# 54rt1n/shardmerge

Hardware: AMD Instinct MI355X
Metric: merged-weight GB/s per GPU + % HBM roofline, Llama-3-70B 3-way FFT merge (higher is better)
Workload: dtype f32; 1 GPU; Llama-3-70B block tensors, this rank's 1/8 slice (9 per block x 10 blocks), K=3 finetunes, bf16 in/out, resident in HBM; workload_id=llama3-70b-slice, k=3, parallelism=tensor-partition x1 (no data-path collective), streams_per_gpu=8

## Files before the change

### shardmerge_amd/csrc/sm_capi.inc

```

struct smhip_ctx {
    smhip::Pipeline<SM_BACKEND> pipe;
    explicit smhip_ctx(int device) : pipe(device) {}
};

#define SM_GUARD(ctx)                      \
    if (!(ctx)) return SMHIP_ERR_ARG;      \
    (ctx)->pipe.err.clear();
#define SM_FINISH(ctx, rc)                                                        \
    do {                                                                          \
        int rc__ = (rc);                                                          \
        if (rc__ == SMHIP_OK && !(ctx)->pipe.be.ok()) {                           \
            (ctx)->pipe.err = (ctx)->pipe.be.error();                             \
            rc__ = SMHIP_ERR_HIP;                                                 \
        }                                                                         \
        return rc__;                                                              \
    } while (0)

template <class Desc, class Scalars>
static int delta_tensor_check(smhip_ctx* ctx, const char* op, const Desc* d, const void* out, const float* delta_out,
                              bool need_base, Scalars scalars) {
    auto bad = [&](const char* what) { return ctx->pipe.fail(SMHIP_ERR_ARG, std::string(op) + ": " + what); };
    if (!d) return bad("null descriptor");
    if (d->k < 1 || d->k > SMHIP_MAX_MODELS) return bad("k out of range (1..16)");
// ... 336 lines not shown
    SM_GUARD(ctx);
    if (!x || !norm_out) return ctx->pipe.fail(SMHIP_ERR_ARG, "bad argument");
    if (dtype < SMHIP_BF16 || dtype > SMHIP_F32) return ctx->pipe.fail(SMHIP_ERR_ARG, "bad dtype");
    ctx->pipe.stream = stream;
    const int rc0 = ctx->pipe.reserve(1, 1);
    if (rc0) SM_FINISH(ctx, rc0);
    smhip::SigDesc sg{x, base, dtype, 1.f};
    double out = 0;
    if (!ctx->pipe.run_serial_norms(&sg, 1, n, &out))
        return ctx->pipe.fail(SMHIP_ERR_ARG, "reference_cpu norm: inputs must be 16-byte aligned");
    *norm_out = (float)out;
    SM_FINISH(ctx, SMHIP_OK);
}

int smhip_debug_option(smhip_ctx* ctx, const char* key, long value) {
    SM_GUARD(ctx);
    if (key && std::string(key) == "aten_overlap") { ctx->pipe.aten_overlap = value != 0; return SMHIP_OK; }
    if (key && std::string(key) == "emf_max_sample") { ctx->pipe.emf_max_sample = value >= 1 && value <= 4096 ? (int)value : smhip::EMF_MAX_SAMPLE; return SMHIP_OK; }
    if (key && std::string(key) == "aten_serial") { ctx->pipe.aten_serial = value != 0; return SMHIP_OK; }
    if (key && std::string(key) == "class_norms") { ctx->pipe.class_norms_mode = value >= 0 && value <= 2 ? (int)value : 1; return SMHIP_OK; }
    if (key && std::string(key) == "cand_cap") { ctx->pipe.debug_cand_cap = value > 0 ? (uint32_t)value : 0u; return SMHIP_OK; }
    if (key && std::string(key) == "sel_chunks") { ctx->pipe.debug_sel_chunks = value > 0 ? (uint32_t)value : 0u; return SMHIP_OK; }
    if (key && std::string(key) == "sel_flush_always") { ctx->pipe.debug_flush_always = value != 0; return SMHIP_OK; }
    if (key && std::string(key) == "fuse_norms") { ctx->pipe.fuse_norms = value != 0; return SMHIP_OK; }
    if (key && std::string(key) == "noise_seed") { ctx->pipe.noise_seed_base = (uint32_t)value; return SMHIP_OK; }
    if (key && std::string(key) == "spectral_intermediates") { ctx->pipe.spectral_inter = value != 0; return SMHIP_OK; }
    if (key && std::string(key) == "fuse_spec_norm") { ctx->pipe.fuse_spec_norm = value != 0; return SMHIP_OK; }
    if (key && std::string(key) == "sel_wgs_per_cu") { ctx->pipe.sel_wgs_per_cu = value > 0 ? (int)value : 5; return SMHIP_OK; }
    if (key && std::string(key) == "pair1d") { ctx->pipe.pair1d_enabled = value != 0; return SMHIP_OK; }
    if (key && std::string(key) == "spec_cull") { ctx->pipe.spec_cull = value != 0; return SMHIP_OK; }
    if (key && std::string(key) == "spec_min_bins") { ctx->pipe.spec_min_bins = value >= 0 ? (size_t)value : (size_t)1 << 20; return SMHIP_OK; }
    if (key && std::string(key) == "dftp_pairs") { ctx->pipe.dftp_pairs_enabled = value != 0; return SMHIP_OK; }
    if (key && std::string(key) == "f2s_pair") { ctx->pipe.f2s_pair = value != 0; return SMHIP_OK; }
    if (key && std::string(key) == "f1_multi") { ctx->pipe.f1_multi = value != 0; return SMHIP_OK; }
    if (key && std::string(key) == "force_bluestein") { ctx->pipe.debug_force_bluestein = value != 0; return SMHIP_OK; }
    if (key && std::string(key) == "force_split") { ctx->pipe.debug_force_split = value > 1 && value <= smhip::DFTP_MAX_P ? (int)value : 0; return SMHIP_OK; }
    if (key && std::string(key) == "fold_columns") { ctx->pipe.fold_enabled = value != 0; return SMHIP_OK; }
    if (key && std::string(key) == "della_slab_rows") { ctx->pipe.della_slab_rows = value > 0 ? (size_t)value : 0; return SMHIP_OK; }
    if (key && std::string(key) == "fold_min_rows") { ctx->pipe.fold_min_rows = value > 0 ? (int)value : SM_FOLD_MIN_ROWS; return SMHIP_OK; }
    return ctx->pipe.fail(SMHIP_ERR_ARG, "unknown debug option");
}

int smhip_debug_query(smhip_ctx* ctx, const char* key, long* value) {
    SM_GUARD(ctx);
    if (!key || !value) return SMHIP_ERR_ARG;
    if (std::string(key) == "spec_hit") { *value = ctx->pipe.last_spec_verdict(); SM_FINISH(ctx, SMHIP_OK); }
    if (std::string(key) == "spec_checked" || std::string(key) == "spec_hits") {
        unsigned long long c = 0, h = 0;
        ctx->pipe.spec_totals(&c, &h);
        *value = (long)(std::string(key) == "spec_hits" ? h : c);
        SM_FINISH(ctx, SMHIP_OK);
    }
    if (std::string(key) == "aten_fast" || std::string(key) == "aten_group" || std::string(key) == "aten_slow") {
        unsigned long long v3[3];
        ctx->pipe.aten_stats(1, v3);
        *value = (long)v3[std::string(key) == "aten_fast" ? 0 : std::string(key) == "aten_group" ? 1 : 2];
        SM_FINISH(ctx, SMHIP_OK);
    }
    return ctx->pipe.fail(SMHIP_ERR_ARG, "unknown debug query");
}

int smhip_profile_enable(smhip_ctx* ctx, int on) { SM_GUARD(ctx); ctx->pipe.be.profile_enable(on != 0); return SMHIP_OK; }
int smhip_profile_reset(smhip_ctx* ctx) { SM_GUARD(ctx); ctx->pipe.be.profile_reset(); return SMHIP_OK; }
int smhip_profile_count(smhip_ctx* ctx) { return ctx ? ctx->pipe.be.profile_count() : 0; }
int smhip_profile_get(smhip_ctx* ctx, int i, const char** name, uint64_t* launches, double* total_ms) {
    SM_GUARD(ctx);
    return ctx->pipe.be.profile_get(i, name, launches, total_ms) ? SMHIP_OK : SMHIP_ERR_ARG;
}

}
```

### shardmerge_amd/csrc/sm_kernels.hpp

```cpp
#pragma once
#include <cmath>
#include <cstring>

#include "fft_engine.hpp"
#include "sm_aten_core.hpp"

namespace smhip {

struct cf4 { float x, y, z, w; };
struct u32x4 { uint32_t x, y, z, w; };

enum { DT_BF16 = 0, DT_F16 = 1, DT_F32 = 2 };

struct SigDesc {
    const void* x;
    const void* base;
    int dtype;
    float prescale;
};

SM_HD uint32_t umax(uint32_t a, uint32_t b) { return a > b ? a : b; }
SM_HD float u2f(uint32_t u) { float f; memcpy(&f, &u, 4); return f; }
SM_HD uint32_t f2u(float f) { uint32_t u; memcpy(&u, &f, 4); return u; }
SM_HD float bf16_to_f(uint32_t h) { return u2f(h << 16); }
// ... 882 lines not shown
    }
}

#ifndef SM_COL_THREADS
#define SM_COL_THREADS 512
#endif
constexpr int f2_bins_for(int T, int N = 1 << 30) {
    if (T == 64 && N <= 256) return 8;
    return (SM_COL_THREADS / (2 * T)) > 1 ? (SM_COL_THREADS / (2 * T) > 8 ? 8 : SM_COL_THREADS / (2 * T)) : 1;
}
#ifndef SM_I1_THREADS
constexpr int i1_bins_for(int T) { return 2; }
#else
constexpr int i1_bins_for(int T) { return (SM_I1_THREADS / T) > 2 ? ((SM_I1_THREADS / T) > 16 ? 16 : (SM_I1_THREADS / T)) : 2; }
#endif
template <class P> constexpr int f2_bins() { if constexpr (P::is_static) return f2_bins_for(P::T, P::N); else return 1; }
template <class P> constexpr int i1_bins() { if constexpr (P::is_static) return i1_bins_for(P::T); else return 2; }

struct F2SParams {
    FftPlanDev plan;
    const cf4* t1;
    int pitch4;
    int R, C, Cb;
    int role_a;
    float scale;
    float* re; float* im;
    unsigned long long* hist;
    int slab, Cb_real, Rfull;
    size_t slab_elems;
    double* im_partials;
    SliceGrid sl;
    int two;
    const cf4* t1_2; int role_a_2; float scale_2; float* re_2;
};
template <class P> constexpr int f2s_groups() {
    if constexpr (P::is_static) return f2_nsig_for(P::T) == 2 ? 2 * f2_bins_for(P::T, P::N) : 1; else return 1;
}

#ifndef SM_F2S_ILV
#define SM_F2S_ILV 1
#endif
constexpr int F2S_ILV = SM_F2S_ILV;
#ifndef SM_F2S_DIRECT
#define SM_F2S_DIRECT 0
#endif
template <class P, int G> constexpr int f2s_direct() {
    if constexpr (!P::is_static) return 0;
    else {
        constexpr int R0 = P::radix(0);
        constexpr bool ok = F2S_ILV == 1 && (G == 1 || G == 2) && P::npass >= 2 && P::T % 2 == 0 && R0 % 2 == 0 &&
                            (P::N / R0) % 2 == 0 && (EMAX / R0) * R0 * P::T >= P::N;
        return ok ? (SM_F2S_DIRECT & 3) : 0;
    }
}
template <class P, int G, bool FOLD = false, class Ex>
SM_HD void k_f2s(Ex& ex, const F2SParams& p) {
    if constexpr (FOLD && !fold_col_plan<P>()) { return; } else {
    typename Ex::template State<FftState> st;
    ex.init(st);
    float* lds = ex.lds() + LDS_SCRATCH_FLOATS;
    const FftPlanDev& pl = p.plan;
    const int T = plan_T<P>(pl), R = plan_N<P>(pl);
    const int LF = plan_lds<P>(pl);
    constexpr int XG = G >= 8 ? 1 : 8 / G;
    int bid_in_slice;
    const int slice = slice_of(ex, p.sl, bid_in_slice);
    int sig2 = 0;
    const int lbid = p.two ? pick_signal(2, bid_in_slice, XG, sig2) : xcd_remap(bid_in_slice, XG);
    const cf4* const t1 = (sig2 ? p.t1_2 : p.t1) + slice * p.sl.t1_stride;
    const size_t pl_off = slice * p.sl.plane_stride;
    const int role_a_ = sig2 ? p.role_a_2 : p.role_a;
    const float scale_ = sig2 ? p.scale_2 : p.scale;
    float* const re_ = sig2 ? p.re_2 : p.re;
    const int kbase = lbid * G;
    if (kbase >= p.Cb) {
        if (p.im_partials) ex.each(st, [&](int tid, FftState&) { if (tid == 0) p.im_partials[ex.bid()] = 0.0; });
        return;
    }
    const int nthreads = G * T;
    const int half = R / 2;
    uint32_t* lhist = (uint32_t*)(lds + G * LF);

    constexpr int DIRECT = f2s_direct<P, G>();
    if constexpr ((DIRECT & 1) != 0) {
        constexpr int R0 = P::radix(0), MB0 = EMAX / R0, nb0 = P::N / R0;
        ex.each(st, [&](int tid, FftState& s) {
            const int g = tid / T, t = tid % T;
            const int k2 = kbase + g;
            const int kc = k2 < p.Cb ? k2 : p.Cb - 1;
            const int par = t & 1;
            static_for<0, MB0>([&](auto m_c) {
                constexpr int m = decltype(m_c)::value;
                const bool live = (t + m * T) < nb0 && k2 < p.Cb;
                static_for<0, R0 / 2>([&](auto q_c) {
                    constexpr int q = decltype(q_c)::value;
                    const int pm = live ? (t >> 1) + m * (T / 2) + q * nb0 + par * (nb0 / 2) : 0;
                    cf4 v;
#if defined(SM_DIAG_NOMEM)
                    v = cf4{(float)q, (float)t, 1.f, (float)kc};
#else
                    if constexpr (FOLD) v = t1[(size_t)(kc / p.slab) * p.slab_elems + (size_t)pm * p.slab + (kc % p.slab)];
                    else v = t1[(size_t)pm * p.pitch4 + kc];
#endif
                    s.xr[m * R0 + 2 * q] = live ? v.x : 0.f; s.xi[m * R0 + 2 * q] = live ? v.y : 0.f;
                    s.xr[m * R0 + 2 * q + 1] = live ? v.z : 0.f; s.xi[m * R0 + 2 * q + 1] = live ? v.w : 0.f;
                });
// ... 55 lines not shown
#pragma unroll
                for (int c = 0; c < 4; ++c) {
                    const int k1 = 4 * (t + u * T) + c;
                    if (k1 < R) o[4 * u + c] = l[lpad(k1)];
                }
            }
        });

    ex.each(st, [&](int tid, FftState& s) {
        const int g = tid / T, t = tid % T;
        const int k2 = kbase + g;
        s.red[0] = 0.0;
        if (k2 >= p.Cb) return;
        const float sc = scale_;
        size_t poff = (size_t)k2 * R;
        int kreal = k2;
        if constexpr (FOLD) { kreal = fold_bin(k2, p.slab, p.Cb_real, R, p.Rfull, poff); if (kreal < 0) return; }
        const uint32_t w = (uint32_t)bin_weight(kreal, p.C);
        float* dre = re_ + pl_off + poff;
        float* dim = p.im + pl_off + poff;
        float imsq = 0.f;
        if constexpr ((DIRECT & 2) != 0) {
            constexpr int RL = P::radix(P::npass - 1), MBL = EMAX / RL, NsL = P::N / RL;
            static_for<0, MBL>([&](auto m_c) {
                constexpr int m = decltype(m_c)::value;
                const int j = t + m * T;
                if (j < NsL) {
                    static_for<0, RL>([&](auto i_c) {
                        constexpr int i = decltype(i_c)::value, e = m * RL + i;
                        const float vr = s.xr[e] * sc;
#if defined(SM_DIAG_NOMEM)
                        if (vr == 12345.678f)
#endif
                        dre[j + i * NsL] = vr;
                        if (role_a_) {
                            const float vi = s.xi[e] * sc;
#if defined(SM_DIAG_NOMEM)
                            if (vi == 12345.678f)
#endif
                            dim[j + i * NsL] = vi;
                            imsq += vi * vi;
                        }
                        if (p.hist) ex.lds_atomic_add(&lhist[(f2u(vr) & 0x7fffffffu) >> 20], w);
                    });
                }
            });
        } else
#pragma unroll
        for (int u = 0; u < EMAX / 4; ++u) {
            const int k0 = 4 * (t + u * T);
            if (k0 + 3 < R && (R & 3) == 0) {
                cf4 vr = {s.xr[4 * u] * sc, s.xr[4 * u + 1] * sc, s.xr[4 * u + 2] * sc, s.xr[4 * u + 3] * sc};
#if defined(SM_DIAG_NOMEM)
                if (vr.x == 12345.678f)
#endif
                *(cf4*)(dre + k0) = vr;
                if (role_a_) {
                    cf4 vi = {s.xi[4 * u] * sc, s.xi[4 * u + 1] * sc, s.xi[4 * u + 2] * sc, s.xi[4 * u + 3] * sc};
#if defined(SM_DIAG_NOMEM)
                    if (vi.x == 12345.678f)
#endif
                    *(cf4*)(dim + k0) = vi;
                    imsq += vi.x * vi.x + vi.y * vi.y + vi.z * vi.z + vi.w * vi.w;
                }
            } else {
#pragma unroll
                for (int c = 0; c < 4; ++c) {
                    if (k0 + c < R) {
                        dre[k0 + c] = s.xr[4 * u + c] * sc;
                        if (role_a_) { const float vi = s.xi[4 * u + c] * sc; dim[k0 + c] = vi; imsq += vi * vi; }
                    }
                }
            }
            if (p.hist) {
#pragma unroll
                for (int c = 0; c < 4; ++c) {
                    if (k0 + c < R) {
                        const uint32_t key = f2u(s.xr[4 * u + c] * sc) & 0x7fffffffu;
                        ex.lds_atomic_add(&lhist[key >> 20], w);
                    }
                }
            }
        }
        s.red[0] = (double)imsq * (double)w;
    });
    if (p.hist) {
        ex.sync();
        ex.each(st, [&](int tid, FftState&) {
            for (int h = tid; h < HIST1_BINS; h += nthreads) {
                const uint32_t v = lhist[h];
                if (v) ex.global_atomic_add(&p.hist[h], (unsigned long long)v);
            }
        });
    }
    if (p.im_partials) {
        ex.sync();
        ex.template block_sum<1>(st, [&](const double* tot) { p.im_partials[ex.bid()] = tot[0]; });
    }
    }
}

template <class Ex>
SM_HD void k_f2_r1(Ex& ex, const F2Params& p) {
// ... 2747 lines not shown
```

### shardmerge_amd/csrc/sm_pipeline.hpp

```cpp
#pragma once
#include <algorithm>
#include <cmath>
#include <cstdio>
#include <map>
#include <string>
#include <vector>

#include "../../include/shardmerge_hip.h"
#include "sm_kernels.hpp"
#include "sm_aten_norm.hpp"
#include "sm_bluestein.hpp"
#include "sm_lora.hpp"
#include "sm_ties.hpp"
#include "sm_dare.hpp"
#include "sm_breadcrumbs.hpp"
#include "sm_geo.hpp"
#include "sm_sce.hpp"
#include "sm_della.hpp"

namespace smhip {

#define SM_KERNEL_TAG(Tag, ParamsT, NAME, CALL)                                      \
    struct Tag {                                                                     \
        using Params = ParamsT;                                                      \
// ... 289 lines not shown
};

struct ProfEntry { std::string name; uint64_t launches = 0; double ms = 0; };

inline size_t round_up(size_t v, size_t m) { return (v + m - 1) / m * m; }

struct PairOut {
    void* out = nullptr; int out_mode = OUT_F32;
    const void* base = nullptr; int base_dtype = DT_BF16;
    float post = 1.f;
    int ifft_policy = 1;
};

template <class B>
class Pipeline {
  public:
    B be;
    std::string err;
    void* stream = nullptr;
    uint32_t debug_cand_cap = 0;
    uint32_t debug_sel_chunks = 0;
    bool debug_flush_always = false;
    bool spec_cull = true;
    size_t spec_min_bins = 1 << 20;
    bool dftp_pairs_enabled = true;
    int debug_force_split = 0;
    int sel_wgs_per_cu = 5;
    bool safe_select = false;
    uint32_t noise_seed_base = 0;
    bool spectral_inter = true;
    bool f2s_pair = true;
    size_t f2s_pair_max_bins = (size_t)64 << 20;
    bool f1_multi = true;
    bool fuse_spec_norm = true;
    float noise_sigma = 1.2e-7f;

    explicit Pipeline(int device) : be(device) {}
    ~Pipeline() {
        for (auto& kv : plans_) if (kv.second.dev.tw) be.free((void*)kv.second.dev.tw);
        for (Buffer* b : {&cand_, &t1_, &small_, &tmpA_, &tmpB_, &tmpC_, &fullS_, &saveR_, &saveI_, &aten_, &emf_, &lora_, &dora_, &ties_}) if (b->p) be.free(b->p);
        for (Buffer& b : pool_) if (b.p) be.free(b.p);
        if (mail_) be.free_host(mail_);
        for (Buffer& b : inter_) if (b.p) be.free(b.p);
        for (Buffer& b : rowspec_) if (b.p) be.free(b.p);
        for (Buffer& b : tr_) if (b.p) be.free(b.p);
        for (auto& kv : rough_tw_) if (kv.second) be.free(kv.second);
        for (auto& kv : blue_) { if (kv.second.chirp) be.free(kv.second.chirp); if (kv.second.filt) be.free(kv.second.filt); }
    }

    int fail(int code, const std::string& msg) { err = msg; return code; }

    int get_plan(int N, FftPlanDev& out) {
        auto it = plans_.find(N);
        if (it == plans_.end()) {
            HostPlan hp;
            int T;
            std::vector<int> rad;
            if (plan_shape(N, T, rad)) {
                hp.ok = true;
                hp.dev.N = N; hp.dev.T = T; hp.dev.npass = (int)rad.size();
                for (int i = 0; i < MAX_PASSES; ++i) hp.dev.radix[i] = i < (int)rad.size() ? rad[i] : 1;
                hp.dev.cx = plan_uses_cx(N) ? 1 : 0;
                hp.dev.lds_floats = hp.dev.cx ? (int)round_up((size_t)2 * (N + (N >> 4) + 1), 32)
                                              : (int)round_up((size_t)lpad(N) + 1, 32);
                std::vector<cf2> tw(N);
                for (int j = 0; j < N; ++j) {
// ... 383 lines not shown
            return SMHIP_OK;
        }
        const int xgs = p.ilv > p.nb ? p.ilv / p.nb : 1;
        const bool joint = joint_rows(g);
        const int nlaunch = joint ? 1 : g.batch;
        if (joint) p.R = g.R * g.rough / 2;
        const int grid = (int)round_up((size_t)(p.R + p.nb - 1) / p.nb, 8 * xgs);
        if (multi && (nlaunch != 1 || g.rough > 1 || (size_t)grid * 2 * nm > PART_DOUBLES || !p.vec)) return SMHIP_ERR_ARG;
        if ((size_t)grid * 2 * nlaunch > PART_DOUBLES) return fail(SMHIP_ERR_SHAPE, "too many rows");
        const size_t lds = (LDS_SCRATCH_FLOATS + (size_t)p.nb * p.plan.lds_floats) * 4;
        cf4* const t1base = p.t1;
        double* const pbase = p.partials;
        if (multi) {
            for (int i = 0; i < nm; ++i) multi->partials[i] = pbase + (size_t)i * 2 * grid;
            multi->b_off = (long long)((size_t)g.C * dt_size(sig.dtype));
            p.sigs = *multi;
            launch_fft<KF1>(p.plan, grid * nm, p.nb * p.plan.T, lds, p, true);
            if (grid_out) *grid_out = grid;
            return SMHIP_OK;
        }
        for (int bi = 0; bi < nlaunch; ++bi) {
            p.a = sig_at(a, (size_t)bi * g.R * g.C); p.b = sig_at(b, (size_t)bi * g.R * g.C);
            p.t1 = t1base + (size_t)bi * (g.t1_slice / 2);
            p.partials = pbase + (size_t)bi * 2 * grid;
            if (blue) { F1BParams q; q.f = p; q.bt = bt; launch_fft<KF1B>(p.plan, grid, p.plan.T, lds, q); }
            else launch_fft<KF1>(p.plan, grid, p.nb * p.plan.T, lds, p, p.vec != 0);
        }
        if (grid_out) *grid_out = grid * nlaunch;
        if (g.rough > 1) return run_dftp(g, t1base, true, F2S_ILV, g.pitch4, g.t1_slice / 2, false);
        return SMHIP_OK;
    }
    struct F2SSecond { const void* t1; bool role_a; float scale; };
    int run_f2s(const Geo& g, bool role_a, float scale, bool hist, const void* t1buf = nullptr, int* im_parts = nullptr,
                const F2SSecond* second = nullptr) {
        F2SParams p;
        p.two = 0; p.t1_2 = nullptr; p.role_a_2 = 0; p.scale_2 = 0.f; p.re_2 = nullptr;
        if (second) {
            if (g.batch != 1 || second->role_a == role_a) return fail(SMHIP_ERR_ARG, "internal: paired column pass");
            p.two = 1; p.t1_2 = (const cf4*)second->t1; p.role_a_2 = second->role_a ? 1 : 0; p.scale_2 = second->scale;
            p.re_2 = plane(g, second->role_a ? P_REA : P_REB);
        }
        const int nsg = second ? 2 : 1;
        const int Rt = g.R / g.fold;
        int rc = get_plan(Rt, p.plan);
        if (rc) return rc;
        p.t1 = (const cf4*)(t1buf ? t1buf : t1_.p); p.pitch4 = g.pitch4 * g.fold; p.R = Rt; p.C = g.C;
        p.Cb = g.fold == 4 ? 4 * g.pitch4 : g.C / 2 + 1;
        p.slab = g.pitch4; p.Cb_real = g.C / 2 + 1; p.Rfull = g.R; p.slab_elems = fold_slab_elems(g, true);
        p.role_a = role_a ? 1 : 0; p.scale = scale;
        p.re = plane(g, role_a ? P_REA : P_REB); p.im = plane(g, P_IMA);
        p.hist = hist ? d_hist() : nullptr;
        const bool st = is_static_plan(p.plan);
        const int G = st ? (f2_nsig_for(p.plan.T) == 2 ? 2 * f2_bins_for(p.plan.T, p.plan.N) : 1) : 1;
        const int xg = G >= 8 ? 1 : 8 / G;
        const int grid = (int)round_up((size_t)(p.Cb + G - 1) / G, 8 * xg) * nsg;
        const size_t lds = (LDS_SCRATCH_FLOATS + (size_t)G * p.plan.lds_floats + HIST1_BINS) * 4;
        const bool any_a = role_a || (second && second->role_a);
        const bool want_im = im_parts && any_a && (size_t)grid * g.batch <= PART_IM_DOUBLES;
        if (im_parts) *im_parts = want_im ? grid * g.batch : -1;
        p.im_partials = want_im ? d_part_im() : nullptr;
        if (g.fold == 4) { launch_fft<KF2SQ>(p.plan, grid, G * p.plan.T, lds, p); return SMHIP_OK; }
        if (g.batch > 1) { p.sl.wgs = grid; p.sl.t1_stride = g.t1_slice / 2; p.sl.plane_stride = (size_t)(g.C / 2 + 1) * g.R; }
        launch_fft<KF2S>(p.plan, grid * g.batch, G * p.plan.T, lds, p);
        return SMHIP_OK;
    }
    void run_spec_norm(const Geo& g, const float* re, const float* im, const float* thr, double& sre, double& sim) {
        const size_t total = (size_t)g.Cb * g.R;
        SpecNormParams q;
        q.re = re; q.im = im; q.R = g.R; q.C = g.Cw; q.Cb = g.Cb; q.vec4 = vec4(g); q.thr = thr;
        q.chunks = pick_chunks((total + 3) / 4, 256, 8, 8);
        int grid = stream_grid((total + 3) / 4, 256, q.chunks);
        while ((size_t)grid * 2 > PART_DOUBLES) { q.chunks *= 2; grid = stream_grid((total + 3) / 4, 256, q.chunks); }
        q.partials = d_part();
        be.template launch<KSpecNorm>(grid, 256, LDS_SCRATCH_FLOATS * 4, q, stream);
        SumPartialsParams sp;
        sp.partials = d_part(); sp.nparts = grid; sp.out = mail_->norm2;
        be.template launch<KSumPartials>(1, 1024, LDS_SCRATCH_FLOATS * 4, sp, stream);
        PublishParams pp;
        pp.flags = d_flags(); pp.thr = d_thr(0); pp.consts = d_consts(); pp.mail = mail_; pp.zero_flags = nullptr;
        be.template launch<KPublish>(1, 64, LDS_SCRATCH_FLOATS * 4, pp, stream);
        be.sync(stream);
        sre = mail_->norm2[0]; sim = mail_->norm2[1];
    }
    void run_spec_rescale(const Geo& g, const float* re, const float* im, float thr, float scale, bool role_a, bool hist,
                          int* im_parts = nullptr) {
        const size_t total = (size_t)g.Cb * g.R;
        SpecRescaleParams q;
        q.re = re; q.im = role_a ? im : nullptr;
        q.dre = plane(g, role_a ? P_REA : P_REB); q.dim = plane(g, P_IMA);
        q.R = g.R; q.C = g.Cw; q.Cb = g.Cb; q.vec4 = vec4(g);
        q.thr = thr; q.scale = scale; q.sigma = noise_sigma; q.seed = ++noise_seed_;
        q.hist = hist ? d_hist() : nullptr;
        q.chunks = pick_chunks((total + 3) / 4, 256, 8, 8);
// ... 533 lines not shown
        std::vector<char> used(m, 0);
        std::vector<float> corr((size_t)m * m, 0.f);
        for (int i = 0; i < m; ++i)
            for (int j = i + 1; j < m; ++j) corr[(size_t)i * m + j] = norms[i] * norms[j];
        for (;;) {
            float best = INFINITY;
            bool any = false;
            for (int i = 0; i < m; ++i)
                for (int j = i + 1; j < m; ++j)
                    if (!used[i] && !used[j]) { any = true; best = std::min(best, std::fabs(corr[(size_t)i * m + j])); }
            if (!any) break;
            int bx = -1, by = -1;
            for (int i = 0; i < m && bx < 0; ++i)
                for (int j = i + 1; j < m; ++j)
                    if (!used[i] && !used[j] && std::fabs(corr[(size_t)i * m + j]) == best) { bx = i; by = j; break; }
            if (bx < 0) break;
            out.emplace_back(bx, by);
            used[bx] = used[by] = 1;
        }
        for (int i = 0; i < m; ++i)
            if (!used[i]) out.emplace_back(i, -1);
    }

    struct Slot {
        SigDesc sig;
        double weight;
        double norm;
        bool spectral = false;
        int re_id = -1, im_id = -1;
        float thr = 0.f;
        double spec_scale = 1.0;
        double post = 1.0;
        int rows_id = -1;
    };
    int materialise(const Geo& g, Slot& s, std::vector<char>& inter_busy) {
        if (!s.spectral) return SMHIP_OK;
        const size_t n = (size_t)g.R * g.C;
        int id = -1;
        for (size_t q = 0; q < inter_.size(); ++q) if (!inter_busy[q]) { id = (int)q; break; }
        if (id < 0) { inter_.emplace_back(); inter_busy.push_back(0); id = (int)inter_.size() - 1; }
        int rc = ensure(inter_[id], n * sizeof(float));
        if (rc) return rc;
        inter_busy[id] = 1;
        PairOut po;
        po.out = inter_[id].p; po.out_mode = OUT_F32; po.post = (float)s.post;
        if ((rc = run_inverse(g, (const float*)pool_[s.re_id].p, (const float*)pool_[s.im_id].p, nullptr, po, nullptr, s.thr))) return rc;
        pool_release(s.re_id); pool_release(s.im_id);
        s.spectral = false; s.re_id = s.im_id = -1;
        s.sig = SigDesc{inter_[id].p, nullptr, DT_F32, 1.f};
        return SMHIP_OK;
    }

    bool run_delta_norms(const smhip_layer_desc& d, size_t n, std::vector<Slot>& stack) {
        if (d.k > NORMS_K || d.in_dtype == DT_F32 || (n % 8) != 0) return false;
        DeltaNormsParams p;
        p.k = d.k; p.dtype = d.in_dtype; p.n = n;
        p.ubase[0] = p.ubase[1] = nullptr;
        int nb = 0;
        for (int i = 0; i < NORMS_K; ++i) { p.ft[i] = d.finetune[i < d.k ? i : 0]; p.base_of[i] = 0; }
        for (int i = 0; i < d.k; ++i) {
            if (!d.base[i] || !aligned16(d.base[i]) || !aligned16(d.finetune[i])) return false;
            int j = 0;
            while (j < nb && p.ubase[j] != d.base[i]) ++j;
            if (j == nb) { if (nb == 2) return false; p.ubase[nb++] = d.base[i]; }
            p.base_of[i] = j;
        }
        p.chunks = pick_chunks(n / 8, 256, 4, 8);
        int grid = stream_grid(n / 8, 256, p.chunks);
        while ((size_t)grid * NORMS_MAX > PART_DOUBLES) { p.chunks *= 2; grid = stream_grid(n / 8, 256, p.chunks); }
        p.partials = d_part();
        be.template launch<KDeltaNorms>(grid, 256, LDS_SCRATCH_FLOATS * 4, p, stream);
        SumNParams sp;
        sp.partials = d_part(); sp.nparts = grid; sp.out = mail_->norm2;
        be.template launch<KSumPartialsN>(1, 256, LDS_SCRATCH_FLOATS * 4, sp, stream);
        be.sync(stream);
        for (int i = 0; i < d.k; ++i) stack[i].norm = std::sqrt(mail_->norm2[i]);
        return true;
    }
// ... 404 lines not shown
                char buf[96];
                snprintf(buf, sizeof buf, "||finetune[%d] - base[%d]|| = %g", i, i, (double)norms32[i]);
                check_flags(false, false);
                return fail(SMHIP_ERR_NONFINITE, buf);
            }
        }
        {
            float acc = 0.f;
            for (int i = 0; i < d.k; ++i) acc += norms32[i];
            mean = (double)(acc / (float)d.k);
        }
        const double target_norm = mean + d.target_norm_offset;
        rp.target_norm = target_norm;
        double cull_pct = d.cull_start_pct;

        std::vector<char> inter_busy(inter_.size(), 0);
        for (size_t q = 0; q < pool_.size(); ++q) {
            bool working = false;
            for (int i = 0; i < 4; ++i) working = working || pidx_[i] == (int)q;
            pool_busy_[q] = working ? 1 : 0;
        }
        noise_seed_ = noise_seed_base;
        int step = 0;
        int round_idx = 0;
        int pair_idx = 0;
        int deferred_step = -1;
        bool deferred_cut = false, deferred_cull = false;
        while (stack.size() > 1) {
            const int m = (int)stack.size();
            std::vector<std::pair<int, int>> pairs;
            correlated_pairs_least(norms32, m, pairs);
            std::vector<Slot> next;
            const bool last_round = (pairs.size() == 1 && pairs[0].second >= 0);
            bool any_pair = false;
            for (auto& pr : pairs) any_pair = any_pair || pr.second >= 0;
            if (!any_pair) { check_flags(false, false); return fail(SMHIP_ERR_NONFINITE, "no pair can be formed (non-finite norms)"); }
            for (auto& pr : pairs) {
                const int x = pr.first, y = pr.second;
                if (step < SMHIP_MAX_PAIRS) { rp.step_x[step] = x; rp.step_y[step] = y; }
                if (y < 0) {
                    next.push_back(stack[x]);
                    if (step < SMHIP_MAX_PAIRS) rp.step_branch[step] = SMHIP_BRANCH_CARRY;
                    ++step;
                    continue;
                }
                Slot A = stack[x], Bs = stack[y];
                const double a_w = stack[x].weight, b_w = stack[y].weight;
                if (A.norm < 0 || Bs.norm < 0) return fail(SMHIP_ERR_ARG, "internal: norm unknown");
                double na = (double)(float)A.norm, nb = (double)(float)Bs.norm;
                bool swapped = false;
                if (std::fabs(na) < std::fabs(nb)) { std::swap(A, Bs); std::swap(na, nb); swapped = true; }
                const double ca = std::fabs(na / target_norm), cb = std::fabs(nb / target_norm);
                const double ratio = cb / (ca + 1e-10);
                PairOut po;
                float* inter = nullptr;
                const bool linear = (nb / (na + 1e-10)) < d.b;
                const bool slerp_proper = !(ca < 1e-6) && !(cb < 1e-6 || ratio < 0.1) && !(nb < 1e-4 || na < 1e-4) && !linear;
                if (last_round) {
                    po = fin;
                } else if (slerp_proper && spectral_ok) {
                } else {
                    int id = -1;
                    for (size_t q = 0; q < inter_.size(); ++q) if (!inter_busy[q]) { id = (int)q; break; }
                    if (id < 0) { inter_.emplace_back(); inter_busy.push_back(0); id = (int)inter_.size() - 1; }
                    Buffer* bb = &inter_[id];
                    if ((rc = ensure(*bb, n * sizeof(float)))) return rc;
                    inter_busy[id] = 1;
                    inter = (float*)bb->p;
// ... 26 lines not shown
                    pa.ifft_policy = 0;
                    if ((rc = pair_arith(A.sig, Bs.sig, R, C, (float)s, (float)(w * s), 1.0, 1, pa, na, nb, &g))) return rc;
                    if (dtmp) {
                        SigDesc ds{dtmp, nullptr, DT_F32, 1.f}, none{nullptr, nullptr, DT_F32, 1.f};
                        run_combine(ds, none, 1.f, 0.f, n, nullptr, &fin, false);
                    }
                    f1_ready = false;
                } else {
                    branch = SMHIP_BRANCH_SLERP;
                    const double t = a_w / (a_w + b_w);
                    if (nb < 1e-4 || na < 1e-4) {
                        SigDesc none{nullptr, nullptr, DT_F32, 1.f};
                        const float sc = (float)(target_norm / na);
                        if (last_round) run_combine(A.sig, none, sc, 0.f, n, delta_out, &po, false);
                        else run_combine(A.sig, none, sc, 0.f, n, inter, nullptr, false);
                        branch = SMHIP_BRANCH_EARLY_V0;
                    } else if (linear) {
                        branch = SMHIP_BRANCH_LINEAR;
                        int grid;
                        if ((rc = run_f1(g, A.sig, Bs.sig, grid))) return rc;
                        f1_ready = false;
                        if ((rc = run_f2_linear(g, (float)(1.0 / na), (float)(1.0 / nb), (float)t))) return rc;
                        PairOut ps = po;
                        ps.post = (float)target_norm;
                        float* dtmp = nullptr;
                        if (last_round && delta_out) { ps = PairOut(); ps.out = delta_out; ps.post = (float)target_norm; dtmp = delta_out; }
                        if ((rc = run_inverse(g, plane(g, P_RER), plane(g, P_IMA), nullptr, ps, last_round ? nullptr : &inv_grid))) return rc;
                        if (dtmp) {
                            SigDesc ds{dtmp, nullptr, DT_F32, 1.f}, none{nullptr, nullptr, DT_F32, 1.f};
                            run_combine(ds, none, 1.f, 0.f, n, nullptr, &fin, false);
                        }
                    } else {
                        int im_parts = -1;
                        const bool any_spec = stack[x].spectral || stack[y].spectral ||
                                              (stack[x].rows_id >= 0 && stack[y].rows_id >= 0);
                        const bool fused1d = !any_spec && pair1d_ok(g);
                        if (fused1d) {
                            f1_ready = false;
                        } else if (!any_spec) {
                            if (!(f1_ready && d.k == 2)) {
                                int grid;
                                if ((rc = run_f1(g, stack[x].sig, stack[y].sig, grid))) return rc;
                            }
                            f1_ready = false;
                            const float s0 = (float)(1.0 / (double)(float)stack[x].norm);
                            const float s1 = (float)(1.0 / (double)(float)stack[y].norm);
                            if ((rc = run_f2(g, s0, s1, swapped ? 1 : 0, d.cutoff_pct > 0))) return rc;
                        } else {
                            f1_ready = false;
                            int* imp = (!last_round && spectral_ok && fuse_spec_norm) ? &im_parts : nullptr;
                            if (f2s_pair && g.batch == 1 && g.fold == 1 && (size_t)g.Cb * g.R <= f2s_pair_max_bins &&
                                !stack[x].spectral && !stack[y].spectral &&
                                stack[x].rows_id >= 0 && stack[y].rows_id >= 0) {
                                const bool xa = !swapped;
                                F2SSecond sec{rowspec_[stack[y].rows_id].p, !xa, (float)(1.0 / (double)(float)stack[y].norm)};
                                if ((rc = run_f2s(g, xa, (float)(1.0 / (double)(float)stack[x].norm), d.cutoff_pct > 0,
                                                  rowspec_[stack[x].rows_id].p, imp, &sec))) return rc;
                            } else
                            for (int side = 0; side < 2; ++side) {
                                const Slot& in = side == 0 ? stack[x] : stack[y];
                                const bool role_a = (side == 0) != swapped;
                                int* ip = role_a ? imp : nullptr;
                                if (in.spectral) {
                                    run_spec_rescale(g, (const float*)pool_[in.re_id].p, (const float*)pool_[in.im_id].p, in.thr,
                                                     (float)in.spec_scale, role_a, d.cutoff_pct > 0, ip);
                                } else if (in.rows_id >= 0) {
                                    if ((rc = run_f2s(g, role_a, (float)(1.0 / (double)(float)in.norm), d.cutoff_pct > 0,
                                                      rowspec_[in.rows_id].p, ip))) return rc;
                                } else {
                                    if ((rc = run_f1_rowpairs(g, in.sig))) return rc;
                                    if ((rc = run_f2s(g, role_a, (float)(1.0 / (double)(float)in.norm), d.cutoff_pct > 0, nullptr, ip))) return rc;
                                }
                            }
                        }
                        bool have_cull;
                        int sel_parts = 0;
                        const bool fused_norm = im_parts > 0 && !safe_select && cull_pct > 0;
                        if (fused1d) have_cull = cull_pct > 0;
                        else spectral_blend(g, BLEND_SLERP, t, d.t_sum, d.cutoff_pct, cull_pct, 1, true, have_cull,
                                            fused_norm ? &sel_parts : nullptr, std::min(pair_idx++, 6));
                        for (int side = 0; side < 2; ++side) {
                            Slot& in = side == 0 ? stack[x] : stack[y];
                            if (in.spectral) { pool_release(in.re_id); pool_release(in.im_id); in.re_id = in.im_id = -1; }
                        }
                        if (!last_round && spectral_ok) {
                            double sre, sim;
                            if (fused_norm && sel_parts > 0) run_spec_norm_fused(sel_parts, im_parts, sre, sim);
                            else run_spec_norm(g, plane(g, P_RER), plane(g, P_IMA), have_cull ? d_thr(1) : nullptr, sre, sim);
                            read_blend_info(&info, d.cutoff_pct > 0, have_cull, true, true);
                            const double ssum = (sre + sim) / ((double)R * (double)C);
                            out_spectral = true;
                            spec_slot = Slot();
                            spec_slot.spectral = true;
                            spec_slot.re_id = pidx_[P_RER]; spec_slot.im_id = pidx_[P_IMA];
                            spec_slot.thr = have_cull ? mail_->thr[1] : 0.f;
                            const double nrm_exact = target_norm * std::sqrt(ssum);
                            const double bias = ref_norms ? aten_gauss_norm_ratio((double)n, nrm_exact / std::sqrt((double)n)) : 1.0;
                            spec_slot.spec_scale = ssum > 0 ? 1.0 / (std::sqrt(ssum) * bias) : 1.0;
                            spec_slot.post = target_norm;
                            spec_slot.norm = nrm_exact * bias;
                            spec_slot.sig = SigDesc{nullptr, nullptr, DT_F32, 1.f};
                            const int r1 = pool_acquire(g.plane_floats * sizeof(float));
                            const int r2 = pool_acquire(g.plane_floats * sizeof(float));
                            if (r1 < 0 || r2 < 0) return SMHIP_ERR_NOMEM;
                            pidx_[P_RER] = r1; pidx_[P_IMA] = r2;
                        } else {
                        PairOut ps = po;
                        ps.post = (float)target_norm;
                        float* dtmp = nullptr;
                        if (last_round && delta_out) { ps = PairOut(); ps.out = delta_out; ps.post = (float)target_norm; dtmp = delta_out; }
                        if (fused1d) {
                            if ((rc = run_pair1d(g, A.sig, Bs.sig, na, nb, t, d.t_sum, d.cutoff_pct, cull_pct, ps,
                                                 last_round ? nullptr : &inv_grid))) return rc;
                        } else
                        if ((rc = run_inverse(g, plane(g, P_RER), plane(g, P_IMA), have_cull ? d_thr(1) : nullptr, ps,
                                              last_round ? nullptr : &inv_grid))) return rc;
                        if (dtmp) {
                            SigDesc ds{dtmp, nullptr, DT_F32, 1.f}, none{nullptr, nullptr, DT_F32, 1.f};
                            run_combine(ds, none, 1.f, 0.f, n, nullptr, &fin, false);
                        }
                        if (last_round) {
                            deferred_step = step; deferred_cut = d.cutoff_pct > 0; deferred_cull = have_cull;
                        } else {
                            read_blend_info(&info, d.cutoff_pct > 0, have_cull, true);
                        }
                        }
                    }
// ... 757 lines not shown
```

Before: 87.26 GB/s.

## Defer storing the Im spectral plane when the slot is carried to the next round

```diff
diff --git a/shardmerge_amd/csrc/sm_capi.inc b/shardmerge_amd/csrc/sm_capi.inc
--- a/shardmerge_amd/csrc/sm_capi.inc
+++ b/shardmerge_amd/csrc/sm_capi.inc
@@ -392,6 +392,7 @@
     if (key && std::string(key) == "spec_min_bins") { ctx->pipe.spec_min_bins = value >= 0 ? (size_t)value : (size_t)1 << 20; return SMHIP_OK; }
     if (key && std::string(key) == "dftp_pairs") { ctx->pipe.dftp_pairs_enabled = value != 0; return SMHIP_OK; }
     if (key && std::string(key) == "f2s_pair") { ctx->pipe.f2s_pair = value != 0; return SMHIP_OK; }
+    if (key && std::string(key) == "lazy_im") { ctx->pipe.lazy_im = value != 0; return SMHIP_OK; }
     if (key && std::string(key) == "f1_multi") { ctx->pipe.f1_multi = value != 0; return SMHIP_OK; }
     if (key && std::string(key) == "force_bluestein") { ctx->pipe.debug_force_bluestein = value != 0; return SMHIP_OK; }
     if (key && std::string(key) == "force_split") { ctx->pipe.debug_force_split = value > 1 && value <= smhip::DFTP_MAX_P ? (int)value : 0; return SMHIP_OK; }
@@ -417,6 +418,8 @@
         *value = (long)v3[std::string(key) == "aten_fast" ? 0 : std::string(key) == "aten_group" ? 1 : 2];
         SM_FINISH(ctx, SMHIP_OK);
     }
+    if (std::string(key) == "lazy_im_skipped") { *value = (long)ctx->pipe.lazy_im_skipped_; SM_FINISH(ctx, SMHIP_OK); }
+    if (std::string(key) == "lazy_im_regenerated") { *value = (long)ctx->pipe.lazy_im_regenerated_; SM_FINISH(ctx, SMHIP_OK); }
     return ctx->pipe.fail(SMHIP_ERR_ARG, "unknown debug query");
 }
 
diff --git a/shardmerge_amd/csrc/sm_kernels.hpp b/shardmerge_amd/csrc/sm_kernels.hpp
--- a/shardmerge_amd/csrc/sm_kernels.hpp
+++ b/shardmerge_amd/csrc/sm_kernels.hpp
@@ -938,6 +938,7 @@
     SliceGrid sl;
     int two;
     const cf4* t1_2; int role_a_2; float scale_2; float* re_2;
+    int store_im, store_im_2, im_only;
 };
 template <class P> constexpr int f2s_groups() {
     if constexpr (P::is_static) return f2_nsig_for(P::T) == 2 ? 2 * f2_bins_for(P::T, P::N) : 1; else return 1;
@@ -978,6 +979,8 @@
     const int role_a_ = sig2 ? p.role_a_2 : p.role_a;
     const float scale_ = sig2 ? p.scale_2 : p.scale;
     float* const re_ = sig2 ? p.re_2 : p.re;
+    const bool store_im_ = (sig2 ? p.store_im_2 : p.store_im) != 0;
+    const bool store_re_ = p.im_only == 0;
     const int kbase = lbid * G;
     if (kbase >= p.Cb) {
         if (p.im_partials) ex.each(st, [&](int tid, FftState&) { if (tid == 0) p.im_partials[ex.bid()] = 0.0; });
@@ -1099,13 +1102,13 @@
 #if defined(SM_DIAG_NOMEM)
                         if (vr == 12345.678f)
 #endif
-                        dre[j + i * NsL] = vr;
+                        if (store_re_) dre[j + i * NsL] = vr;
                         if (role_a_) {
                             const float vi = s.xi[e] * sc;
 #if defined(SM_DIAG_NOMEM)
                             if (vi == 12345.678f)
 #endif
-                            dim[j + i * NsL] = vi;
+                            if (store_im_) dim[j + i * NsL] = vi;
                             imsq += vi * vi;
                         }
                         if (p.hist) ex.lds_atomic_add(&lhist[(f2u(vr) & 0x7fffffffu) >> 20], w);
@@ -1121,21 +1124,21 @@
 #if defined(SM_DIAG_NOMEM)
                 if (vr.x == 12345.678f)
 #endif
-                *(cf4*)(dre + k0) = vr;
+                if (store_re_) *(cf4*)(dre + k0) = vr;
                 if (role_a_) {
                     cf4 vi = {s.xi[4 * u] * sc, s.xi[4 * u + 1] * sc, s.xi[4 * u + 2] * sc, s.xi[4 * u + 3] * sc};
 #if defined(SM_DIAG_NOMEM)
                     if (vi.x == 12345.678f)
 #endif
-                    *(cf4*)(dim + k0) = vi;
+                    if (store_im_) *(cf4*)(dim + k0) = vi;
                     imsq += vi.x * vi.x + vi.y * vi.y + vi.z * vi.z + vi.w * vi.w;
                 }
             } else {
 #pragma unroll
                 for (int c = 0; c < 4; ++c) {
                     if (k0 + c < R) {
-                        dre[k0 + c] = s.xr[4 * u + c] * sc;
-                        if (role_a_) { const float vi = s.xi[4 * u + c] * sc; dim[k0 + c] = vi; imsq += vi * vi; }
+                        if (store_re_) dre[k0 + c] = s.xr[4 * u + c] * sc;
+                        if (role_a_) { const float vi = s.xi[4 * u + c] * sc; if (store_im_) dim[k0 + c] = vi; imsq += vi * vi; }
                     }
                 }
             }
diff --git a/shardmerge_amd/csrc/sm_pipeline.hpp b/shardmerge_amd/csrc/sm_pipeline.hpp
--- a/shardmerge_amd/csrc/sm_pipeline.hpp
+++ b/shardmerge_amd/csrc/sm_pipeline.hpp
@@ -345,6 +345,8 @@
     bool f2s_pair = true;
     size_t f2s_pair_max_bins = (size_t)64 << 20;
     bool f1_multi = true;
+    bool lazy_im = true;
+    unsigned long long lazy_im_skipped_ = 0, lazy_im_regenerated_ = 0;
     bool fuse_spec_norm = true;
     float noise_sigma = 1.2e-7f;
 
@@ -794,9 +796,11 @@
     }
     struct F2SSecond { const void* t1; bool role_a; float scale; };
     int run_f2s(const Geo& g, bool role_a, float scale, bool hist, const void* t1buf = nullptr, int* im_parts = nullptr,
-                const F2SSecond* second = nullptr) {
+                const F2SSecond* second = nullptr, bool* skip_im = nullptr, float* im_only_dst = nullptr) {
         F2SParams p;
         p.two = 0; p.t1_2 = nullptr; p.role_a_2 = 0; p.scale_2 = 0.f; p.re_2 = nullptr;
+        p.store_im = p.store_im_2 = 1; p.im_only = 0;
+        if (im_only_dst && (!role_a || second || hist || im_parts || skip_im)) return fail(SMHIP_ERR_ARG, "internal: Im-only column pass");
         if (second) {
             if (g.batch != 1 || second->role_a == role_a) return fail(SMHIP_ERR_ARG, "internal: paired column pass");
             p.two = 1; p.t1_2 = (const cf4*)second->t1; p.role_a_2 = second->role_a ? 1 : 0; p.scale_2 = second->scale;
@@ -811,6 +815,7 @@
         p.slab = g.pitch4; p.Cb_real = g.C / 2 + 1; p.Rfull = g.R; p.slab_elems = fold_slab_elems(g, true);
         p.role_a = role_a ? 1 : 0; p.scale = scale;
         p.re = plane(g, role_a ? P_REA : P_REB); p.im = plane(g, P_IMA);
+        if (im_only_dst) { p.im_only = 1; p.re = im_only_dst; p.im = im_only_dst; }
         p.hist = hist ? d_hist() : nullptr;
         const bool st = is_static_plan(p.plan);
         const int G = st ? (f2_nsig_for(p.plan.T) == 2 ? 2 * f2_bins_for(p.plan.T, p.plan.N) : 1) : 1;
@@ -821,6 +826,10 @@
         const bool want_im = im_parts && any_a && (size_t)grid * g.batch <= PART_IM_DOUBLES;
         if (im_parts) *im_parts = want_im ? grid * g.batch : -1;
         p.im_partials = want_im ? d_part_im() : nullptr;
+        if (skip_im) {
+            *skip_im = *skip_im && want_im;
+            if (*skip_im) { if (role_a) p.store_im = 0; else p.store_im_2 = 0; }
+        }
         if (g.fold == 4) { launch_fft<KF2SQ>(p.plan, grid, G * p.plan.T, lds, p); return SMHIP_OK; }
         if (g.batch > 1) { p.sl.wgs = grid; p.sl.t1_stride = g.t1_slice / 2; p.sl.plane_stride = (size_t)(g.C / 2 + 1) * g.R; }
         launch_fft<KF2S>(p.plan, grid * g.batch, G * p.plan.T, lds, p);
@@ -1420,7 +1429,16 @@
         double spec_scale = 1.0;
         double post = 1.0;
         int rows_id = -1;
+        int im_rows_id = -1;
+        float im_scale = 0.f;
     };
+    int regenerate_im(const Geo& g, Slot& s) {
+        if (!s.spectral || s.im_rows_id < 0) return SMHIP_OK;
+        int rc = run_f2s(g, true, s.im_scale, false, rowspec_[s.im_rows_id].p, nullptr, nullptr, nullptr, (float*)pool_[s.im_id].p);
+        ++lazy_im_regenerated_;
+        s.im_rows_id = -1;
+        return rc;
+    }
     int materialise(const Geo& g, Slot& s, std::vector<char>& inter_busy) {
         if (!s.spectral) return SMHIP_OK;
         const size_t n = (size_t)g.R * g.C;
@@ -1432,6 +1450,7 @@
         inter_busy[id] = 1;
         PairOut po;
         po.out = inter_[id].p; po.out_mode = OUT_F32; po.post = (float)s.post;
+        if ((rc = regenerate_im(g, s))) return rc;
         if ((rc = run_inverse(g, (const float*)pool_[s.re_id].p, (const float*)pool_[s.im_id].p, nullptr, po, nullptr, s.thr))) return rc;
         pool_release(s.re_id); pool_release(s.im_id);
         s.spectral = false; s.re_id = s.im_id = -1;
@@ -1902,8 +1921,8 @@
             correlated_pairs_least(norms32, m, pairs);
             std::vector<Slot> next;
             const bool last_round = (pairs.size() == 1 && pairs[0].second >= 0);
-            bool any_pair = false;
-            for (auto& pr : pairs) any_pair = any_pair || pr.second >= 0;
+            bool any_pair = false, round_carries = false;
+            for (auto& pr : pairs) { any_pair = any_pair || pr.second >= 0; round_carries = round_carries || pr.second < 0; }
             if (!any_pair) { check_flags(false, false); return fail(SMHIP_ERR_NONFINITE, "no pair can be formed (non-finite norms)"); }
             for (auto& pr : pairs) {
                 const int x = pr.first, y = pr.second;
@@ -1996,6 +2015,8 @@
                         }
                     } else {
                         int im_parts = -1;
+                        int lazy_rows = -1;
+                        float lazy_scale = 0.f;
                         const bool any_spec = stack[x].spectral || stack[y].spectral ||
                                               (stack[x].rows_id >= 0 && stack[y].rows_id >= 0);
                         const bool fused1d = !any_spec && pair1d_ok(g);
@@ -2013,29 +2034,34 @@
                         } else {
                             f1_ready = false;
                             int* imp = (!last_round && spectral_ok && fuse_spec_norm) ? &im_parts : nullptr;
+                            Slot& in_a = swapped ? stack[y] : stack[x];
+                            bool skip_im = lazy_im && round_carries && imp && !safe_select && cull_pct > 0 && !in_a.spectral &&
+                                           in_a.rows_id >= 0;
                             if (f2s_pair && g.batch == 1 && g.fold == 1 && (size_t)g.Cb * g.R <= f2s_pair_max_bins &&
                                 !stack[x].spectral && !stack[y].spectral &&
                                 stack[x].rows_id >= 0 && stack[y].rows_id >= 0) {
                                 const bool xa = !swapped;
                                 F2SSecond sec{rowspec_[stack[y].rows_id].p, !xa, (float)(1.0 / (double)(float)stack[y].norm)};
                                 if ((rc = run_f2s(g, xa, (float)(1.0 / (double)(float)stack[x].norm), d.cutoff_pct > 0,
-                                                  rowspec_[stack[x].rows_id].p, imp, &sec))) return rc;
+                                                  rowspec_[stack[x].rows_id].p, imp, &sec, &skip_im))) return rc;
                             } else
                             for (int side = 0; side < 2; ++side) {
-                                const Slot& in = side == 0 ? stack[x] : stack[y];
+                                Slot& in = side == 0 ? stack[x] : stack[y];
                                 const bool role_a = (side == 0) != swapped;
                                 int* ip = role_a ? imp : nullptr;
                                 if (in.spectral) {
+                                    if (role_a && (rc = regenerate_im(g, in))) return rc;
                                     run_spec_rescale(g, (const float*)pool_[in.re_id].p, (const float*)pool_[in.im_id].p, in.thr,
                                                      (float)in.spec_scale, role_a, d.cutoff_pct > 0, ip);
                                 } else if (in.rows_id >= 0) {
                                     if ((rc = run_f2s(g, role_a, (float)(1.0 / (double)(float)in.norm), d.cutoff_pct > 0,
-                                                      rowspec_[in.rows_id].p, ip))) return rc;
+                                                      rowspec_[in.rows_id].p, ip, nullptr, role_a ? &skip_im : nullptr))) return rc;
                                 } else {
                                     if ((rc = run_f1_rowpairs(g, in.sig))) return rc;
                                     if ((rc = run_f2s(g, role_a, (float)(1.0 / (double)(float)in.norm), d.cutoff_pct > 0, nullptr, ip))) return rc;
                                 }
                             }
+                            if (skip_im) { lazy_rows = in_a.rows_id; lazy_scale = (float)(1.0 / (double)(float)in_a.norm); }
                         }
                         bool have_cull;
                         int sel_parts = 0;
@@ -2050,6 +2076,7 @@
                         if (!last_round && spectral_ok) {
                             double sre, sim;
                             if (fused_norm && sel_parts > 0) run_spec_norm_fused(sel_parts, im_parts, sre, sim);
+                            else if (lazy_rows >= 0) return fail(SMHIP_ERR_ARG, "internal: the Parseval pass needs an Im plane that was not stored");
                             else run_spec_norm(g, plane(g, P_RER), plane(g, P_IMA), have_cull ? d_thr(1) : nullptr, sre, sim);
                             read_blend_info(&info, d.cutoff_pct > 0, have_cull, true, true);
                             const double ssum = (sre + sim) / ((double)R * (double)C);
@@ -2057,6 +2084,8 @@
                             spec_slot = Slot();
                             spec_slot.spectral = true;
                             spec_slot.re_id = pidx_[P_RER]; spec_slot.im_id = pidx_[P_IMA];
+                            spec_slot.im_rows_id = lazy_rows; spec_slot.im_scale = lazy_scale;
+                            if (lazy_rows >= 0) ++lazy_im_skipped_;
                             spec_slot.thr = have_cull ? mail_->thr[1] : 0.f;
                             const double nrm_exact = target_norm * std::sqrt(ssum);
                             const double bias = ref_norms ? aten_gauss_norm_ratio((double)n, nrm_exact / std::sqrt((double)n)) : 1.0;
```

Result: faster. 88.16 GB/s, median of 6 (+1.0%).
